# zhangxiaochen95/uav_bs_ctrl

Hardware: AMD Instinct MI355X
Metric: env-steps/sec (MADRQN, 8 UBS x 80 GT) (higher is better)
Workload: dtype f32

## Files before the change

### uav_bs_ctrl_amd/csrc/gatv2_bwd_mfma.hip

```cpp
#define UAVGNN_GATV2_BWD_MFMA_TU 1
#include <type_traits>

#include "gatv2.hip"

namespace uavgnn {
namespace {

__device__ __forceinline__ float readlane_f(float v, int l) {
  return __uint_as_float(__builtin_amdgcn_readlane(__float_as_uint(v), l));
}
__device__ __forceinline__ void wave_totals16(const float (&v)[16], float (&t)[4]) {
  float w[8];
#pragma unroll
  for (int i = 0; i < 8; ++i) {
    const auto s = __builtin_amdgcn_permlane32_swap(__float_as_uint(v[i]), __float_as_uint(v[i + 8]), false, false);
    w[i] = __uint_as_float(s[0]) + __uint_as_float(s[1]);
  }
#pragma unroll
  for (int i = 0; i < 4; ++i) {
    const auto s = __builtin_amdgcn_permlane16_swap(__float_as_uint(w[i]), __float_as_uint(w[i + 4]), false, false);
    t[i] = row16_allsum(__uint_as_float(s[0]) + __uint_as_float(s[1]));
  }
}

__device__ __forceinline__ K1Split k1_split_pair(float a, float b) {
  K1Split s;
  s.h1 = __builtin_bit_cast(unsigned, __builtin_convertvector(k1_f32x2{a, b}, k1_bf16x2));
  const float a1 = a - __uint_as_float(s.h1 << 16), b1 = b - __uint_as_float(s.h1 & 0xffff0000u);
  s.h2 = __builtin_bit_cast(unsigned, __builtin_convertvector(k1_f32x2{a1, b1}, k1_bf16x2));
  const float a2 = a1 - __uint_as_float(s.h2 << 16), b2 = b1 - __uint_as_float(s.h2 & 0xffff0000u);
  s.h3 = __builtin_bit_cast(unsigned, __builtin_convertvector(k1_f32x2{a2, b2}, k1_bf16x2));
  return s;
}

template <bool LEAN, bool HT>
__global__ __launch_bounds__(kThreads, UAVGNN_BWD_OCC) void gatv2_bwd_resident_kernel(
    const float* __restrict__ x_src, const float* __restrict__ x_dst, const int32_t* __restrict__ seg_off,
    const int32_t* __restrict__ dst_order, int N,
    const float* __restrict__ W_s, const float* __restrict__ b_s, const float* __restrict__ W_d,
    const float* __restrict__ b_d, const float* __restrict__ attn, float slope, const float* __restrict__ out,
    const float* __restrict__ d_out, int ld_out, const float* __restrict__ a_save, float* __restrict__ partial,
    int onepass_max_deg) {
  constexpr int FS = 4, NH = 4, D = 64, H = NH * D, J = H / kWave, CT = H / 16;
  constexpr int P = partial_len<FS>(H);
  constexpr int ES = FS + 2 * NH;
  constexpr int szE = kWavesPerBlock * 2 * kWave * ES * 4, szV = kWavesPerBlock * NH * kWave * 16, szWop = CT * kWave * 16;
  constexpr int szC = (kWavesPerBlock + 1) * CT * 32 * 4, szD = 3 * H * 4;
  constexpr int oE = 0, oV = oE + szE, oWop = oV + szV, oC = oWop + szWop, oD = oC + szC, kLdsBytes = oD + szD;
  static_assert(P * 4 <= szWop, "fold buffer aliases the score operands");
  static_assert(kLdsBytes <= 80 * 1024, "two workgroups per CU");
  static_assert(kWave * 20 * 4 <= 2 * kWave * ES * 4, "the final conversion of the accumulators fits the staging area");
  __shared__ __attribute__((aligned(16))) unsigned char lds[kLdsBytes];
  k1_u32x4* const sWop = reinterpret_cast<k1_u32x4*>(lds + oWop);
  float* const sRed = reinterpret_cast<float*>(lds + oWop);
  float* const sD = reinterpret_cast<float*>(lds + oD);

  const int tid = threadIdx.x;
  const int lane = tid & (kWave - 1);
  const int wave = __builtin_amdgcn_readfirstlane(tid >> 6);
  const int j16 = lane & 15, g4 = lane >> 4;
  const float c_lin = 0.5f * (1.f + slope), c_abs = 0.5f * (1.f - slope);

  for (int i = tid; i < CT * kWave; i += kThreads) {
    const int ct = i >> 6, l = i & 63;
    sWop[i] = k1_a_operand(0.f - W_s[(16 * ct + (l & 15)) * FS + (l >> 4)], 0.f, 0);
  }
  for (int i = tid; i < CT * 32; i += kThreads) reinterpret_cast<unsigned*>(lds + oC)[kWavesPerBlock * CT * 32 + i] = 0u;
  for (int n = tid; n < H; n += kThreads) {
    sD[n] = W_d[2 * n];
    sD[H + n] = W_d[2 * n + 1];
    sD[2 * H + n] = b_d[n] + b_s[n];
  }
  for (int i = lane; i < NH * kWave; i += kWave)
    (reinterpret_cast<k1_u32x4*>(lds + oV) + wave * NH * kWave)[i] = k1_u32x4{0u, 0u, 0u, 0u};

  float Ws[J][FS];
  float aWs[J][FS], aWr0[J], aWr1[J], abr[J], sS1[J], sX0[J], sX1[J];
#pragma unroll
  for (int j = 0; j < J; ++j) {
    const int n = lane + kWave * j;
#pragma unroll
    for (int f = 0; f < FS; ++f) {
      Ws[j][f] = W_s[n * FS + f];
      aWs[j][f] = 0.f;
    }
    aWr0[j] = aWr1[j] = abr[j] = sS1[j] = sX0[j] = sX1[j] = 0.f;
  }
  float accP[FS];
#pragma unroll
  for (int f = 0; f < FS; ++f) accP[f] = 0.f;
  bwd_f32x4 acc[CT];
#pragma unroll
  for (int ct = 0; ct < CT; ++ct) acc[ct] = bwd_f32x4{0.f, 0.f, 0.f, 0.f};
  __syncthreads();

  float* __restrict__ ew = reinterpret_cast<float*>(lds + oE) + wave * 2 * kWave * ES;
  k1_u32x4* __restrict__ vw = reinterpret_cast<k1_u32x4*>(lds + oV) + wave * NH * kWave;
  unsigned* __restrict__ cwt = reinterpret_cast<unsigned*>(lds + oC) + wave * CT * 32;
  const unsigned* __restrict__ cwl = reinterpret_cast<const unsigned*>(lds + oC) +
      (g4 < 2 ? wave * CT * 32 + 16 * g4 + j16 : kWavesPerBlock * CT * 32 + (lane & 31));

  auto load_rows = [&](const int v, float (&o)[J], float (&gr)[J]) {
    const float* __restrict__ orow = out + static_cast<size_t>(v) * ld_out;
    const float* __restrict__ grow = d_out + static_cast<size_t>(v) * ld_out;
#pragma unroll
    for (int j = 0; j < J; ++j) {
      o[j] = orow[lane + kWave * j];
      gr[j] = grow[lane + kWave * j];
    }
  };

  auto process = [&](const float (&o_)[J], const float (&gr_)[J], const int e0, const int deg, const float xv0, const float xv1) {
    float g[J], c[J];
#pragma unroll
    for (int j = 0; j < J; ++j) {
      g[j] = o_[j] > 0.f ? gr_[j] : 0.f;
      aWr0[j] = fmaf(g[j], xv0, aWr0[j]);
      aWr1[j] = fmaf(g[j], xv1, aWr1[j]);
      abr[j] += g[j];
      const int n = lane + kWave * j;
      c[j] = fmaf(sD[H + n], xv1, fmaf(sD[n], xv0, sD[2 * H + n]));
    }
    float G[NH][FS];
    {
      float gv[16], gt[4];
#pragma unroll
      for (int j = 0; j < J; ++j)
#pragma unroll
        for (int f = 0; f < FS; ++f) gv[4 * j + f] = g[j] * Ws[j][f];
      wave_totals16(gv, gt);
#pragma unroll
      for (int k = 0; k < NH; ++k)
#pragma unroll
        for (int f = 0; f < FS; ++f) G[k][f] = readlane_f(gt[f], 16 * k);
    }
    float x[2][FS], a[2][NH], dt[2][NH], t[NH], sb[16];
#pragma unroll
    for (int k = 0; k < NH; ++k) t[k] = 0.f;
#pragma unroll
    for (int m = 0; m < 16; ++m) sb[m] = 0.f;
#pragma unroll
    for (int ch = 0; ch < 2; ++ch) {
      const int slot = ch * kWave + lane;
      if (slot < deg) {
        const int u = e0 + slot;
        load_row<FS>(x_src + static_cast<size_t>(u) * FS, x[ch]);
        load_row<NH>(a_save + static_cast<size_t>(u) * NH, a[ch]);
      } else {
#pragma unroll
        for (int f = 0; f < FS; ++f) x[ch][f] = 0.f;
#pragma unroll
        for (int k = 0; k < NH; ++k) a[ch][k] = 0.f;
      }
    }
#pragma unroll
    for (int ch = 0; ch < 2; ++ch) {
#pragma unroll
      for (int k = 0; k < NH; ++k) {
        float d = 0.f;
#pragma unroll
        for (int f = 0; f < FS; ++f) d = fmaf(G[k][f], x[ch][f], d);
        dt[ch][k] = d;
        t[k] = fmaf(a[ch][k], d, t[k]);
#pragma unroll
        for (int f = 0; f < FS; ++f) sb[4 * k + f] = fmaf(a[ch][k], x[ch][f], sb[4 * k + f]);
      }
      if (ch * kWave < deg)
        *reinterpret_cast<bwd_f32x4*>(ew + (ch * kWave + lane) * ES) = bwd_f32x4{x[ch][0], x[ch][1], x[ch][2], x[ch][3]};
    }
    float T[NH];
#pragma unroll
    for (int k = 0; k < NH; ++k) T[k] = wave_total_dpp(t[k]);
    {
      float st[4];
      wave_totals16(sb, st);
#pragma unroll
      for (int j = 0; j < J; ++j)
#pragma unroll
        for (int f = 0; f < FS; ++f) aWs[j][f] = fmaf(g[j], readlane_f(st[f], 16 * j), aWs[j][f]);
    }
    {
      float pv[16], pt[4];
#pragma unroll
      for (int m = 0; m < 16; ++m) pv[m] = 0.f;
#pragma unroll
      for (int ch = 0; ch < 2; ++ch) {
        float de[NH];
#pragma unroll
        for (int k = 0; k < NH; ++k) {
          de[k] = a[ch][k] * (dt[ch][k] - T[k]);
#pragma unroll
          for (int f = 0; f < FS; ++f) pv[4 * k + f] = fmaf(de[k], x[ch][f], pv[4 * k + f]);
        }
        if (ch * kWave < deg)
          *reinterpret_cast<bwd_f32x4*>(ew + (ch * kWave + lane) * ES + FS) = bwd_f32x4{de[0], de[1], de[2], de[3]};
      }
      wave_totals16(pv, pt);
#pragma unroll
      for (int f = 0; f < FS; ++f) accP[f] += pt[f];
    }
#pragma unroll
    for (int j = 0; j < J; ++j) {
      const K1Split sc = k1_split(0.f - c[j]);
      unsigned* q = cwt + ((lane >> 4) + 4 * j) * 32 + (lane & 15);
      q[0] = (sc.h1 & 0xffffu) | (sc.h2 & 0xffff0000u);
      q[16] = sc.h3 & 0xffffu;
    }
    wave_sync();

    const bwd_f32x4 czero = {0.f, 0.f, 0.f, 0.f};
    unsigned k_sign = 0x80008000u, k_one = 0x3F803F80u;
    asm volatile("" : "+v"(k_sign), "+v"(k_one));
    auto trip = [&](const int tp, auto half_c) {
      constexpr bool HALF = decltype(half_c)::value;
      const float* const et = ew + 32 * tp * ES;
      if constexpr (HALF) {
        int ln = lane;
        asm volatile("" : "+v"(ln));
        const int i16 = ln & 15, h = ln >> 4;
        const float* er = et + i16 * ES;
        const bwd_f32x4 xa = *reinterpret_cast<const bwd_f32x4*>(er);
        const float da = er[FS + h];
        const float va[5] = {da, da * xa[0], da * xa[1], da * xa[2], da * xa[3]};
        const int skew = (i16 >> 2) + 4 * h;
        unsigned short* dst = reinterpret_cast<unsigned short*>(reinterpret_cast<unsigned*>(vw) + (h * kWave + (i16 >> 2) * 16) * 4 +
                                                                ((i16 & 3) >> 1)) + (i16 & 1);
#pragma unroll
        for (int f = 0; f < 5; ++f) {
          const K1Split sa = k1_split(va[f]);
          const int r0 = f == 0 ? 0 : 2 + f, dr = f == 0 ? 1 : 4;
          dst[((r0 + 0 * dr + skew) & 15) * 8] = static_cast<unsigned short>(sa.h1);
          dst[((r0 + 1 * dr + skew) & 15) * 8] = static_cast<unsigned short>(sa.h2);
          dst[((r0 + 2 * dr + skew) & 15) * 8] = static_cast<unsigned short>(sa.h3);
        }
      } else {
        const int ep = lane & 15, h = lane >> 4;
        const int e_a = 2 * ep, i16 = e_a & 15;
        const float* er = et + e_a * ES;
        const bwd_f32x4 xa = *reinterpret_cast<const bwd_f32x4*>(er), xb = *reinterpret_cast<const bwd_f32x4*>(er + ES);
        const float da = er[FS + h], db = er[ES + FS + h];
        const float va[5] = {da, da * xa[0], da * xa[1], da * xa[2], da * xa[3]};
        const float vb[5] = {db, db * xb[0], db * xb[1], db * xb[2], db * xb[3]};
        const int skew = (i16 >> 2) + 4 * h;
        unsigned* dst = reinterpret_cast<unsigned*>(vw) + (h * kWave + (i16 >> 2) * 16) * 4 + (((i16 & 3) + 4 * (e_a >> 4)) >> 1);
#pragma unroll
        for (int f = 0; f < 5; ++f) {
          const int r0 = f == 0 ? 0 : 2 + f, dr = f == 0 ? 1 : 4;
          if constexpr (LEAN) {
            const K1Split sp = k1_split_pair(va[f], vb[f]);
            dst[((r0 + 0 * dr + skew) & 15) * 4] = sp.h1;
            dst[((r0 + 1 * dr + skew) & 15) * 4] = sp.h2;
            dst[((r0 + 2 * dr + skew) & 15) * 4] = sp.h3;
          } else {
            const K1Split sa = k1_split(va[f]), sb2 = k1_split(vb[f]);
            dst[((r0 + 0 * dr + skew) & 15) * 4] = (sa.h1 & 0xffffu) | (sb2.h1 & 0xffff0000u);
            dst[((r0 + 1 * dr + skew) & 15) * 4] = (sa.h2 & 0xffffu) | (sb2.h2 & 0xffff0000u);
            dst[((r0 + 2 * dr + skew) & 15) * 4] = (sa.h3 & 0xffffu) | (sb2.h3 & 0xffff0000u);
          }
        }
      }
      constexpr int NT = HALF ? 1 : 2;
      k1_bf16x8 xop[NT];
#pragma unroll
      for (int tt = 0; tt < NT; ++tt) xop[tt] = k1_b_operand(et[(16 * tt + j16) * ES + g4], 0x3F803F80u);
      wave_sync_lds();
      auto v_operand = [&](const int i) {
        k1_u32x4 v = vw[i];
        if constexpr (HALF) v[2] = v[3] = 0u;
        return v;
      };
      k1_u32x4 vop = v_operand(16 * g4 + ((j16 + g4) & 15)), vop_n = v_operand(kWave + 16 * g4 + ((j16 + g4 + 4) & 15));
      auto w_operand = [&](const int ct_) {
        if constexpr (LEAN) {
          const unsigned* wp = reinterpret_cast<const unsigned*>(sWop + ct_ * kWave + lane);
          const uint2 w01 = *reinterpret_cast<const uint2*>(wp);
          return __builtin_bit_cast(k1_bf16x8, k1_u32x4{w01.x, w01.y, wp[2], cwl[ct_ * 32]});
        }
        k1_u32x4 w = sWop[ct_ * kWave + lane];
        w[3] = cwl[ct_ * 32];
        return __builtin_bit_cast(k1_bf16x8, w);
      };
      k1_bf16x8 w_nn = w_operand(1);
      bwd_f32x4 d0, d1 = czero;
      {
        const k1_bf16x8 w0 = w_operand(0);
        d0 = __builtin_amdgcn_mfma_f32_16x16x32_bf16(xop[0], w0, czero, 0, 0, 0);
        if constexpr (!HALF) d1 = __builtin_amdgcn_mfma_f32_16x16x32_bf16(xop[NT - 1], w0, czero, 0, 0, 0);
      }
      __builtin_amdgcn_sched_barrier(0);
#pragma unroll
      for (int ct = 0; ct < CT; ++ct) {
        bwd_f32x4 e0_ = d0, e1_ = d1;
        if (ct + 1 < CT) {
          e0_ = __builtin_amdgcn_mfma_f32_16x16x32_bf16(xop[0], w_nn, czero, 0, 0, 0);
          if constexpr (!HALF) e1_ = __builtin_amdgcn_mfma_f32_16x16x32_bf16(xop[NT - 1], w_nn, czero, 0, 0, 0);
          if (ct + 2 < CT) w_nn = w_operand(ct + 2);
          __builtin_amdgcn_sched_barrier(0);
        }
        k1_u32x4 sg = {0u, 0u, 0u, 0u};
#pragma unroll
        for (int q = 0; q < 2; ++q) {
          const unsigned p0 = __builtin_amdgcn_perm(__float_as_uint(d0[2 * q + 1]), __float_as_uint(d0[2 * q]), 0x07060302u);
          sg[q] = (p0 & k_sign) | (k_one & ~k_sign);
          if constexpr (!HALF) {
            const unsigned p1 = __builtin_amdgcn_perm(__float_as_uint(d1[2 * q + 1]), __float_as_uint(d1[2 * q]), 0x07060302u);
            sg[2 + q] = (p1 & k_sign) | (k_one & ~k_sign);
          }
        }
        acc[ct] = __builtin_amdgcn_mfma_f32_16x16x32_bf16(__builtin_bit_cast(k1_bf16x8, vop), __builtin_bit_cast(k1_bf16x8, sg),
                                                          acc[ct], 0, 0, 0);
        if ((ct & 3) == 3 && ct + 1 < CT) {
          vop = vop_n;
          if (ct + 5 < CT) vop_n = v_operand(((ct + 5) >> 2) * kWave + 16 * g4 + ((j16 + g4 + 4 * ((ct + 5) >> 2)) & 15));
        }
        __builtin_amdgcn_sched_barrier(0);
        d0 = e0_;
        d1 = e1_;
      }
      wave_sync_lds();
    };
    {
      int tp = 0;
      for (; 32 * tp + (HT ? 16 : 0) < deg; ++tp) trip(tp, std::false_type{});
      if (HT && 32 * tp < deg) trip(tp, std::true_type{});
    }
    float s1[CT];
    const bool s1_lane = lane < 16;
#pragma unroll
    for (int ct = 0; ct < CT; ++ct) {
      const float sum = (acc[ct][0] + acc[ct][1]) + acc[ct][2];
      s1[ct] = LEAN ? sum : -sum;
#pragma unroll
      for (int i = 0; i < 3; ++i) {
        if constexpr (LEAN)
          acc[ct][i] = __uint_as_float(__builtin_amdgcn_update_dpp(__float_as_uint(acc[ct][i]), 0u, 0xE4, 0x1, 0xf, false));
        else
          acc[ct][i] = s1_lane ? 0.f : acc[ct][i];
      }
    }
#pragma unroll
    for (int j = 0; j < J; ++j) {
      const auto r = __builtin_amdgcn_permlane16_swap(__float_as_uint(s1[4 * j]), __float_as_uint(s1[4 * j + 1]), false, false);
      const auto q = __builtin_amdgcn_permlane16_swap(__float_as_uint(s1[4 * j + 2]), __float_as_uint(s1[4 * j + 3]), false, false);
      const auto s = __builtin_amdgcn_permlane32_swap(r[0], q[0], false, false);
      const float S1 = LEAN ? -__uint_as_float(s[0]) : __uint_as_float(s[0]);
      sS1[j] += S1;
      sX0[j] = fmaf(xv0, S1, sX0[j]);
      sX1[j] = fmaf(xv1, S1, sX1[j]);
    }
    wave_sync();
  };

  const int stride = gridDim.x * kWavesPerBlock;
  const int it0 = blockIdx.x * kWavesPerBlock + wave;
  for (int kb = 0; it0 + kb * stride < N; kb += kWave) {
    const int my_it = it0 + (kb + lane) * stride;
    const bool mine = my_it < N;
    const int m_v = mine ? (dst_order ? dst_order[my_it] : my_it) : 0;
    const int m_e0 = mine ? seg_off[m_v] : 0;
    const int m_e1 = mine ? seg_off[m_v + 1] : 0;
    const float2 m_xv = mine ? *reinterpret_cast<const float2*>(x_dst + 2 * m_v) : make_float2(0.f, 0.f);
    const int cnt = min(kWave, (N - it0 - kb * stride + stride - 1) / stride);
    auto in_cls = [&](const int i) {
      const int dg = __builtin_amdgcn_readlane(m_e1, i) - __builtin_amdgcn_readlane(m_e0, i);
      return dg >= kMfMinDeg && dg <= onepass_max_deg;
    };
    float on[J], gn[J];
    int ii = 0;
    while (ii < cnt && !in_cls(ii)) ++ii;
    if (ii < cnt) load_rows(__builtin_amdgcn_readlane(m_v, ii), on, gn);
    while (ii < cnt) {
      float oc[J], gc[J];
#pragma unroll
      for (int j = 0; j < J; ++j) {
        oc[j] = on[j];
        gc[j] = gn[j];
      }
      int nx = ii + 1;
      while (nx < cnt && !in_cls(nx)) ++nx;
      if (nx < cnt) load_rows(__builtin_amdgcn_readlane(m_v, nx), on, gn);
      const int e0 = __builtin_amdgcn_readlane(m_e0, ii);
      process(oc, gc, e0, __builtin_amdgcn_readlane(m_e1, ii) - e0,
              __uint_as_float(__builtin_amdgcn_readlane(__float_as_uint(m_xv.x), ii)),
              __uint_as_float(__builtin_amdgcn_readlane(__float_as_uint(m_xv.y), ii)));
      ii = nx;
    }
  }

  float abs_[J], aWd0[J], aWd1[J], abd[J], aatt[J];
  {
    constexpr int kCvLd = 20;
    int le = lane;
    if constexpr (HT) asm volatile("" : "+v"(le));
    float* __restrict__ cv = ew;
#pragma unroll
    for (int k = 0; k < NH; ++k) {
#pragma unroll
      for (int c4 = 0; c4 < 4; ++c4) *reinterpret_cast<bwd_f32x4*>(cv + (c4 * 16 + j16) * kCvLd + 4 * g4) = acc[4 * k + c4];
      wave_sync_lds();
      float r[16];
#pragma unroll
      for (int q = 0; q < 4; ++q) {
        const bwd_f32x4 t4 = *reinterpret_cast<const bwd_f32x4*>(cv + lane * kCvLd + 4 * q);
        r[4 * q] = t4[0]; r[4 * q + 1] = t4[1]; r[4 * q + 2] = t4[2]; r[4 * q + 3] = t4[3];
      }
      wave_sync_lds();
      const float att = attn[le + kWave * k];
      float wS2 = 0.f, wP = 0.f;
#pragma unroll
      for (int f = 0; f < FS; ++f) {
        const float S2 = -((r[3 + f] + r[7 + f]) + r[11 + f]);
        const float pkf = readlane_f(accP[f], 16 * k);
        wS2 = fmaf(Ws[k][f], S2, wS2);
        wP = fmaf(Ws[k][f], pkf, wP);
        aWs[k][f] = fmaf(att, fmaf(c_abs, S2, c_lin * pkf), aWs[k][f]);
      }
      const int n = lane + kWave * k;
      const float cS1 = fmaf(sD[H + n], sX1[k], fmaf(sD[n], sX0[k], sD[2 * H + n] * sS1[k]));
      aatt[k] = fmaf(c_abs, cS1 + wS2, c_lin * wP);
      const float der = att * c_abs;
      abd[k] = der * sS1[k];
      abs_[k] = abr[k] + abd[k];
      aWd0[k] = der * sX0[k];
      aWd1[k] = der * sX1[k];
    }
  }

  __syncthreads();
  for (int w = 0; w < kWavesPerBlock; ++w) {
    if (wave == w) {
#pragma unroll
      for (int j = 0; j < J; ++j) {
        const int n = lane + kWave * j;
        auto put = [&](int idx, float val) { sRed[idx] = (w == 0) ? val : sRed[idx] + val; };
#pragma unroll
        for (int f = 0; f < FS; ++f) put(n * FS + f, aWs[j][f]);
        int o = H * FS;
        put(o + n, abs_[j]);
        o += H;
        put(o + 2 * n, aWd0[j]);
        put(o + 2 * n + 1, aWd1[j]);
        o += 2 * H;
        put(o + n, abd[j]);
        o += H;
        put(o + n, aatt[j]);
        o += H;
        put(o + 2 * n, aWr0[j]);
        put(o + 2 * n + 1, aWr1[j]);
        o += 2 * H;
        put(o + n, abr[j]);
      }
    }
    __syncthreads();
  }
  float* __restrict__ prow = partial + static_cast<size_t>(blockIdx.x) * P;
  for (int i = tid; i < P; i += kThreads) prow[i] = sRed[i];
}

}

int gatv2_bwd_resident_launch(const float* x_src, const float* x_dst, const int32_t* seg_off, const int32_t* dst_order, int N,
                              const float* W_s, const float* b_s, const float* W_d, const float* b_d, const float* attn, float slope,
                              const float* out, const float* d_out, int ld_out, const float* a_save, float* partial,
                              int onepass_max_deg, int grid, hipStream_t st) {
  if (onepass_max_deg > 2 * kWave) return UAVGNN_EINVAL;
  auto off = [](const char* name) {
    const char* e = getenv(name);
    return e && e[0] == '0';
  };
  const bool lean = !off("UAVGNN_K1_BWD_LEAN"), ht = !off("UAVGNN_K1_BWD_HALFTRIP");
#define UAVGNN_RESIDENT_LAUNCH(LEANV, HTV)                                                                                          \
  hipLaunchKernelGGL((gatv2_bwd_resident_kernel<LEANV, HTV>), dim3(grid), dim3(kThreads), 0, st, x_src, x_dst, seg_off, dst_order, \
                     N, W_s, b_s, W_d, b_d, attn, slope, out, d_out, ld_out, a_save, partial, onepass_max_deg)
  if (lean && ht) UAVGNN_RESIDENT_LAUNCH(true, true);
  else if (lean) UAVGNN_RESIDENT_LAUNCH(true, false);
  else if (ht) UAVGNN_RESIDENT_LAUNCH(false, true);
  else UAVGNN_RESIDENT_LAUNCH(false, false);
#undef UAVGNN_RESIDENT_LAUNCH
  return launch_status();
}
}
```

Measured before the change: 2.650 million.

## Add TRIM variant of resident GATv2 backward with banked wave reductions

Adds a TRIM template variant, enabled by default, of the resident GATv2 backward kernel. It replaces the four-register cross-wave reductions with a single banked register, where lanes hold the different totals. It also packs the cwt split in pairs with byte permutes, changes the V-operand row layout so half trips no longer need zeroing, and prefetches W operands two tiles ahead. The S1 extraction is done with permlane swaps instead of the older path. The aim is fewer reduction instructions and fewer LDS and VALU operations per edge group, at the cost of a more intricate layout that the epilogue indexing must match exactly.

```diff
diff --git a/uav_bs_ctrl_amd/csrc/gatv2_bwd_mfma.hip b/uav_bs_ctrl_amd/csrc/gatv2_bwd_mfma.hip
--- a/uav_bs_ctrl_amd/csrc/gatv2_bwd_mfma.hip
+++ b/uav_bs_ctrl_amd/csrc/gatv2_bwd_mfma.hip
@@ -21,6 +21,40 @@
     const auto s = __builtin_amdgcn_permlane16_swap(__float_as_uint(w[i]), __float_as_uint(w[i + 4]), false, false);
     t[i] = row16_allsum(__uint_as_float(s[0]) + __uint_as_float(s[1]));
   }
+}
+
+__device__ __forceinline__ float wave_totals16_banked(const float (&v)[16]) {
+  float w[8], x[4];
+#pragma unroll
+  for (int i = 0; i < 8; ++i) {
+    const auto s = __builtin_amdgcn_permlane32_swap(__float_as_uint(v[i]), __float_as_uint(v[i + 8]), false, false);
+    w[i] = __uint_as_float(s[0]) + __uint_as_float(s[1]);
+  }
+#pragma unroll
+  for (int i = 0; i < 4; ++i) {
+    const auto s = __builtin_amdgcn_permlane16_swap(__float_as_uint(w[i]), __float_as_uint(w[i + 4]), false, false);
+    x[i] = __uint_as_float(s[0]) + __uint_as_float(s[1]);
+    x[i] += dpp_f<kRowRorCtl + 8>(x[i]);
+    x[i] += dpp_f<kRowRorCtl + 4>(x[i]);
+  }
+  unsigned u = __float_as_uint(x[0]);
+  u = __builtin_amdgcn_update_dpp(u, __float_as_uint(x[1]), 0xE4, 0xf, 0x2, false);
+  u = __builtin_amdgcn_update_dpp(u, __float_as_uint(x[2]), 0xE4, 0xf, 0x4, false);
+  u = __builtin_amdgcn_update_dpp(u, __float_as_uint(x[3]), 0xE4, 0xf, 0x8, false);
+  float t = __uint_as_float(u);
+  t += dpp_f<kQuadXor2Ctl>(t);
+  t += dpp_f<kQuadXor1Ctl>(t);
+  return t;
+}
+__device__ __forceinline__ float wave_totals4(const float (&v)[4]) {
+  float r[4];
+#pragma unroll
+  for (int k = 0; k < 4; ++k) r[k] = row16_allsum(v[k]);
+  const auto a = __builtin_amdgcn_permlane16_swap(__float_as_uint(r[0]), __float_as_uint(r[1]), false, false);
+  const auto b = __builtin_amdgcn_permlane16_swap(__float_as_uint(r[2]), __float_as_uint(r[3]), false, false);
+  const float s01 = __uint_as_float(a[0]) + __uint_as_float(a[1]), s23 = __uint_as_float(b[0]) + __uint_as_float(b[1]);
+  const auto s = __builtin_amdgcn_permlane32_swap(__float_as_uint(s01), __float_as_uint(s23), false, false);
+  return __uint_as_float(s[0]) + __uint_as_float(s[1]);
 }
 
 __device__ __forceinline__ K1Split k1_split_pair(float a, float b) {
@@ -33,7 +67,7 @@
   return s;
 }
 
-template <bool LEAN, bool HT>
+template <bool LEAN, bool HT, bool TRIM = false>
 __global__ __launch_bounds__(kThreads, UAVGNN_BWD_OCC) void gatv2_bwd_resident_kernel(
     const float* __restrict__ x_src, const float* __restrict__ x_dst, const int32_t* __restrict__ seg_off,
     const int32_t* __restrict__ dst_order, int N,
@@ -43,6 +77,7 @@
     int onepass_max_deg) {
   constexpr int FS = 4, NH = 4, D = 64, H = NH * D, J = H / kWave, CT = H / 16;
   constexpr int P = partial_len<FS>(H);
+  static_assert(!TRIM || (LEAN && HT), "TRIM is built on the lean kernel with the half trip");
   constexpr int ES = FS + 2 * NH;
   constexpr int szE = kWavesPerBlock * 2 * kWave * ES * 4, szV = kWavesPerBlock * NH * kWave * 16, szWop = CT * kWave * 16;
   constexpr int szC = (kWavesPerBlock + 1) * CT * 32 * 4, szD = 3 * H * 4;
@@ -128,11 +163,19 @@
       for (int j = 0; j < J; ++j)
 #pragma unroll
         for (int f = 0; f < FS; ++f) gv[4 * j + f] = g[j] * Ws[j][f];
-      wave_totals16(gv, gt);
-#pragma unroll
-      for (int k = 0; k < NH; ++k)
-#pragma unroll
-        for (int f = 0; f < FS; ++f) G[k][f] = readlane_f(gt[f], 16 * k);
+      if constexpr (TRIM) {
+        const float gu = wave_totals16_banked(gv);
+#pragma unroll
+        for (int k = 0; k < NH; ++k)
+#pragma unroll
+          for (int f = 0; f < FS; ++f) G[k][f] = readlane_f(gu, 16 * k + 4 * f);
+      } else {
+        wave_totals16(gv, gt);
+#pragma unroll
+        for (int k = 0; k < NH; ++k)
+#pragma unroll
+          for (int f = 0; f < FS; ++f) G[k][f] = readlane_f(gt[f], 16 * k);
+      }
     }
     float x[2][FS], a[2][NH], dt[2][NH], t[NH], sb[16];
 #pragma unroll
@@ -170,8 +213,17 @@
     }
     float T[NH];
 #pragma unroll
-    for (int k = 0; k < NH; ++k) T[k] = wave_total_dpp(t[k]);
-    {
+    for (int k = 0; k < NH; ++k) T[k] = TRIM ? 0.f : wave_total_dpp(t[k]);
+    if constexpr (TRIM) {
+      const float tt = wave_totals4(t);
+#pragma unroll
+      for (int k = 0; k < NH; ++k) T[k] = readlane_f(tt, 16 * k);
+      const float su = wave_totals16_banked(sb);
+#pragma unroll
+      for (int j = 0; j < J; ++j)
+#pragma unroll
+        for (int f = 0; f < FS; ++f) aWs[j][f] = fmaf(g[j], readlane_f(su, 16 * j + 4 * f), aWs[j][f]);
+    } else {
       float st[4];
       wave_totals16(sb, st);
 #pragma unroll
@@ -195,16 +247,32 @@
         if (ch * kWave < deg)
           *reinterpret_cast<bwd_f32x4*>(ew + (ch * kWave + lane) * ES + FS) = bwd_f32x4{de[0], de[1], de[2], de[3]};
       }
-      wave_totals16(pv, pt);
-#pragma unroll
-      for (int f = 0; f < FS; ++f) accP[f] += pt[f];
-    }
-#pragma unroll
-    for (int j = 0; j < J; ++j) {
-      const K1Split sc = k1_split(0.f - c[j]);
-      unsigned* q = cwt + ((lane >> 4) + 4 * j) * 32 + (lane & 15);
-      q[0] = (sc.h1 & 0xffffu) | (sc.h2 & 0xffff0000u);
-      q[16] = sc.h3 & 0xffffu;
+      if constexpr (TRIM) {
+        accP[0] += wave_totals16_banked(pv);
+      } else {
+        wave_totals16(pv, pt);
+#pragma unroll
+        for (int f = 0; f < FS; ++f) accP[f] += pt[f];
+      }
+    }
+    if constexpr (TRIM) {
+#pragma unroll
+      for (int j = 0; j < J; j += 2) {
+        const K1Split sc = k1_split_pair(0.f - c[j], 0.f - c[j + 1]);
+        unsigned* q = cwt + ((lane >> 4) + 4 * j) * 32 + (lane & 15);
+        q[0] = __builtin_amdgcn_perm(sc.h2, sc.h1, 0x05040100u);
+        q[16] = sc.h3 & 0xffffu;
+        q[4 * 32] = __builtin_amdgcn_perm(sc.h2, sc.h1, 0x07060302u);
+        q[4 * 32 + 16] = sc.h3 >> 16;
+      }
+    } else {
+#pragma unroll
+      for (int j = 0; j < J; ++j) {
+        const K1Split sc = k1_split(0.f - c[j]);
+        unsigned* q = cwt + ((lane >> 4) + 4 * j) * 32 + (lane & 15);
+        q[0] = (sc.h1 & 0xffffu) | (sc.h2 & 0xffff0000u);
+        q[16] = sc.h3 & 0xffffu;
+      }
     }
     wave_sync();
 
@@ -214,7 +282,7 @@
     auto trip = [&](const int tp, auto half_c) {
       constexpr bool HALF = decltype(half_c)::value;
       const float* const et = ew + 32 * tp * ES;
-      if constexpr (HALF) {
+      if constexpr (HALF && !TRIM) {
         int ln = lane;
         asm volatile("" : "+v"(ln));
         const int i16 = ln & 15, h = ln >> 4;
@@ -228,7 +296,7 @@
 #pragma unroll
         for (int f = 0; f < 5; ++f) {
           const K1Split sa = k1_split(va[f]);
-          const int r0 = f == 0 ? 0 : 2 + f, dr = f == 0 ? 1 : 4;
+          const int r0 = f == 0 ? 0 : (TRIM ? 4 * f - 3 : 2 + f), dr = (f == 0) != TRIM ? 1 : 4;
           dst[((r0 + 0 * dr + skew) & 15) * 8] = static_cast<unsigned short>(sa.h1);
           dst[((r0 + 1 * dr + skew) & 15) * 8] = static_cast<unsigned short>(sa.h2);
           dst[((r0 + 2 * dr + skew) & 15) * 8] = static_cast<unsigned short>(sa.h3);
@@ -245,7 +313,7 @@
         unsigned* dst = reinterpret_cast<unsigned*>(vw) + (h * kWave + (i16 >> 2) * 16) * 4 + (((i16 & 3) + 4 * (e_a >> 4)) >> 1);
 #pragma unroll
         for (int f = 0; f < 5; ++f) {
-          const int r0 = f == 0 ? 0 : 2 + f, dr = f == 0 ? 1 : 4;
+          const int r0 = f == 0 ? 0 : (TRIM ? 4 * f - 3 : 2 + f), dr = (f == 0) != TRIM ? 1 : 4;
           if constexpr (LEAN) {
             const K1Split sp = k1_split_pair(va[f], vb[f]);
             dst[((r0 + 0 * dr + skew) & 15) * 4] = sp.h1;
@@ -262,11 +330,11 @@
       constexpr int NT = HALF ? 1 : 2;
       k1_bf16x8 xop[NT];
 #pragma unroll
-      for (int tt = 0; tt < NT; ++tt) xop[tt] = k1_b_operand(et[(16 * tt + j16) * ES + g4], 0x3F803F80u);
+      for (int tt = 0; tt < NT; ++tt) xop[tt] = k1_b_operand(et[(16 * tt + j16) * ES + g4], TRIM ? k_one : 0x3F803F80u);
       wave_sync_lds();
       auto v_operand = [&](const int i) {
         k1_u32x4 v = vw[i];
-        if constexpr (HALF) v[2] = v[3] = 0u;
+        if constexpr (HALF && !TRIM) v[2] = v[3] = 0u;
         return v;
       };
       k1_u32x4 vop = v_operand(16 * g4 + ((j16 + g4) & 15)), vop_n = v_operand(kWave + 16 * g4 + ((j16 + g4 + 4) & 15));
@@ -280,7 +348,7 @@
         w[3] = cwl[ct_ * 32];
         return __builtin_bit_cast(k1_bf16x8, w);
       };
-      k1_bf16x8 w_nn = w_operand(1);
+      k1_bf16x8 w_nn = w_operand(1), w_n2 = w_operand(TRIM ? 2 : 1);
       bwd_f32x4 d0, d1 = czero;
       {
         const k1_bf16x8 w0 = w_operand(0);
@@ -294,7 +362,8 @@
         if (ct + 1 < CT) {
           e0_ = __builtin_amdgcn_mfma_f32_16x16x32_bf16(xop[0], w_nn, czero, 0, 0, 0);
           if constexpr (!HALF) e1_ = __builtin_amdgcn_mfma_f32_16x16x32_bf16(xop[NT - 1], w_nn, czero, 0, 0, 0);
-          if (ct + 2 < CT) w_nn = w_operand(ct + 2);
+          if constexpr (TRIM) w_nn = w_n2;
+          else if (ct + 2 < CT) w_nn = w_operand(ct + 2);
           __builtin_amdgcn_sched_barrier(0);
         }
         k1_u32x4 sg = {0u, 0u, 0u, 0u};
@@ -307,6 +376,10 @@
             sg[2 + q] = (p1 & k_sign) | (k_one & ~k_sign);
           }
         }
+        if constexpr (TRIM) {
+          __builtin_amdgcn_sched_barrier(0);
+          if (ct + 3 < CT) w_n2 = w_operand(ct + 3);
+        }
         acc[ct] = __builtin_amdgcn_mfma_f32_16x16x32_bf16(__builtin_bit_cast(k1_bf16x8, vop), __builtin_bit_cast(k1_bf16x8, sg),
                                                           acc[ct], 0, 0, 0);
         if ((ct & 3) == 3 && ct + 1 < CT) {
@@ -324,6 +397,22 @@
       for (; 32 * tp + (HT ? 16 : 0) < deg; ++tp) trip(tp, std::false_type{});
       if (HT && 32 * tp < deg) trip(tp, std::true_type{});
     }
+    if constexpr (TRIM) {
+#pragma unroll
+      for (int j = 0; j < J; ++j) {
+        const auto r = __builtin_amdgcn_permlane16_swap(__float_as_uint(acc[4 * j][0]), __float_as_uint(acc[4 * j + 1][0]), false, false);
+        const auto q = __builtin_amdgcn_permlane16_swap(__float_as_uint(acc[4 * j + 2][0]), __float_as_uint(acc[4 * j + 3][0]), false, false);
+        const float b01 = __uint_as_float(r[0]) + __uint_as_float(r[1]);
+        const float b23 = __uint_as_float(q[0]) + __uint_as_float(q[1]);
+        const auto s = __builtin_amdgcn_permlane32_swap(__float_as_uint(b01), __float_as_uint(b23), false, false);
+        const float S1 = -(__uint_as_float(s[0]) + __uint_as_float(s[1]));
+        sS1[j] += S1;
+        sX0[j] = fmaf(xv0, S1, sX0[j]);
+        sX1[j] = fmaf(xv1, S1, sX1[j]);
+#pragma unroll
+        for (int r4 = 0; r4 < 4; ++r4) acc[4 * j + r4][0] = 0.f;
+      }
+    } else {
     float s1[CT];
     const bool s1_lane = lane < 16;
 #pragma unroll
@@ -347,6 +436,7 @@
       sS1[j] += S1;
       sX0[j] = fmaf(xv0, S1, sX0[j]);
       sX1[j] = fmaf(xv1, S1, sX1[j]);
+    }
     }
     wave_sync();
   };
@@ -409,8 +499,8 @@
       float wS2 = 0.f, wP = 0.f;
 #pragma unroll
       for (int f = 0; f < FS; ++f) {
-        const float S2 = -((r[3 + f] + r[7 + f]) + r[11 + f]);
-        const float pkf = readlane_f(accP[f], 16 * k);
+        const float S2 = TRIM ? -((r[4 * f + 1] + r[4 * f + 2]) + r[4 * f + 3]) : -((r[3 + f] + r[7 + f]) + r[11 + f]);
+        const float pkf = TRIM ? readlane_f(accP[0], 16 * k + 4 * f) : readlane_f(accP[f], 16 * k);
         wS2 = fmaf(Ws[k][f], S2, wS2);
         wP = fmaf(Ws[k][f], pkf, wP);
         aWs[k][f] = fmaf(att, fmaf(c_abs, S2, c_lin * pkf), aWs[k][f]);
@@ -468,11 +558,12 @@
     const char* e = getenv(name);
     return e && e[0] == '0';
   };
-  const bool lean = !off("UAVGNN_K1_BWD_LEAN"), ht = !off("UAVGNN_K1_BWD_HALFTRIP");
-#define UAVGNN_RESIDENT_LAUNCH(LEANV, HTV)                                                                                          \
-  hipLaunchKernelGGL((gatv2_bwd_resident_kernel<LEANV, HTV>), dim3(grid), dim3(kThreads), 0, st, x_src, x_dst, seg_off, dst_order, \
+  const bool lean = !off("UAVGNN_K1_BWD_LEAN"), ht = !off("UAVGNN_K1_BWD_HALFTRIP"), trim = !off("UAVGNN_K1_BWD_TRIM");
+#define UAVGNN_RESIDENT_LAUNCH(...)                                                                                                  \
+  hipLaunchKernelGGL((gatv2_bwd_resident_kernel<__VA_ARGS__>), dim3(grid), dim3(kThreads), 0, st, x_src, x_dst, seg_off, dst_order, \
                      N, W_s, b_s, W_d, b_d, attn, slope, out, d_out, ld_out, a_save, partial, onepass_max_deg)
-  if (lean && ht) UAVGNN_RESIDENT_LAUNCH(true, true);
+  if (lean && ht && trim) UAVGNN_RESIDENT_LAUNCH(true, true, true);
+  else if (lean && ht) UAVGNN_RESIDENT_LAUNCH(true, true);
   else if (lean) UAVGNN_RESIDENT_LAUNCH(true, false);
   else if (ht) UAVGNN_RESIDENT_LAUNCH(false, true);
   else UAVGNN_RESIDENT_LAUNCH(false, false);
```

Result: no change. 2.667 million, median of 6 (+0.6%).
